# pandegroup/openmm

Hardware: NVIDIA H100
Metric: ns/day (higher is better)
Workload: dtype f32

## Files before the change

### openmm_b200/csrc/engine.cu

```cuda
#include "engine.h"
#include "../../include/b200md.h"
#include <stdexcept>
#include <algorithm>
#include <cmath>
#include <cstring>
#include <cstdlib>
#include <map>
#include <set>
#include <dlfcn.h>
#include <thread>

static std::string g_create_error;

template <class T> struct DevBuf {
    T* p = nullptr; size_t n = 0; bool owned = true;
    void attach(void* ptr, size_t count) { free(); p = (T*) ptr; n = count; owned = false; }
    void alloc(size_t count) {
        if (!owned) { if (count > n) throw std::runtime_error("window buffer too small"); return; }
        free(); n = count; if (count) CUDA_CHECK(cudaMalloc(&p, count*sizeof(T)));
    }
    void upload(const std::vector<T>& v) { if (v.size() > n) alloc(v.size()); if (!v.empty()) CUDA_CHECK(cudaMemcpy(p, v.data(), v.size()*sizeof(T), cudaMemcpyHostToDevice)); }
    void zero() { if (n) CUDA_CHECK(cudaMemset(p, 0, n*sizeof(T))); }
    void free() { if (p && owned) cudaFree(p); p = nullptr; n = 0; owned = true; }
    ~DevBuf() { free(); }
// ... 39 lines not shown
    bool pmeOnly = false;
    bool listDirty = true;
    bool overlapPme = true;
    bool pmeBrick = true;
    int brickAtoms = 64, brickPoints = 8192;
    bool listBuilt = false;
    std::vector<double> mass, charge, sigma, epsilon;
    b200md_nonbonded_desc nbdesc{};
    bool haveNb = false;
    std::vector<int> excI, excJ; std::vector<double> excQQ, excSig, excEps;
    std::vector<int> bondI, bondJ; std::vector<double> bondR0, bondK;
    std::vector<int> angI, angJ, angK; std::vector<double> angT0, angKK;
    std::vector<int> torI, torJ, torK, torL, torN; std::vector<double> torPhase, torKK;
    std::vector<int> rbI, rbJ, rbK, rbL; std::vector<double> rbC;
    std::vector<int> cmapSize, cmapMap, cmapAtoms; std::vector<double> cmapCoeff;
    std::vector<unsigned char> bondGroup, angGroup, torGroup, rbGroup, cmapGroup;
    std::vector<int> conI, conJ; std::vector<double> conD;
    int cmFreq = 0;
    std::vector<int4> hUnitAtoms;
    double boxA[3] = {0, 0, 0}, boxB[3] = {0, 0, 0}, boxC[3] = {0, 0, 0};
    bool haveBox = false;
    bool haveOrigin = false;
    double padFrac = 0.10;
    DevBuf<float4> posq, velm, sposq[2], swrap[2], refPos, atomShift, blockCenter[2], blockHalf[2], superCenter[2], superHalf[2];
    DevBuf<float2> sigeps, ssigeps[2];
    DevBuf<double> chargeD; DevBuf<double2> sigepsD;
    DevBuf<long long> force;
    DevBuf<double> energy, cmScratch;
    DevBuf<int> molStart, molAtoms, cellOffset, sorig[2], sortedOf, cellRank, cellCount, cellFill, atomCell, tmpSorted, tileI[2], tileJ[2], tileMask[2], listCounters, counters, exclStart, exclList;
    DevBuf<unsigned int> maskPool[2];
    DevBuf<unsigned long long> stepCounter;
    DevBuf<unsigned int> blocksDone;
    bool stepStateValid = false;
    DevBuf<real> grid, eterm;
    DevBuf<long long> gridFixed;
    DevBuf<real2> cgrid;
    DevBuf<real2> tw[3];
    DevBuf<double> moduli[3];
    DevBuf<int2> bondAtoms, excAtoms; DevBuf<double2> bondParams, angleParams;
    DevBuf<int4> angleAtoms, torsionAtoms, unitAtoms; DevBuf<double4> torsionParams, excParams;
    DevBuf<int> unitType; DevBuf<float4> unitParams;
    DevBuf<unsigned char> bondGroupDev, angGroupDev, torGroupDev, rbGroupDev, cmapGroupDev;
    DevBuf<int4> rbAtoms, cmapAtomsDev; DevBuf<double> rbParams, cmapCoeffDev; DevBuf<int> cmapMapDev; DevBuf<int2> cmapMapsDev;
    std::vector<int> ccmaCons;
    DevBuf<int> ccCompCon, ccCompAtom, ccRowStart, ccCol, ccAtoms, ccAStart, ccACon;
    DevBuf<int2> ccConAtoms; DevBuf<float> ccDist, ccRedMass, ccVal, ccDelta1, ccDelta2;
    DevBuf<float4> ccRij, ccXold, ccXunc;
    int precision = B200MD_PRECISION_SINGLE;
    DevBuf<float4> posqCorr; DevBuf<double4> velmD, unitParamsD;
    DevBuf<double> ccDistD, ccRedMassD, ccDelta1D, ccDelta2D; DevBuf<double4> ccRijD, ccXoldD, ccXuncD, ccXposD;
    bool mixed() const { return precision == B200MD_PRECISION_MIXED; }
    CcmaDev ccma{};
    NbDev nb{};
    PmeDev pme{};
    BondedDev bd{};
    UnitDev units{};
    IntegDev integ{};
    bool haveIntegrator = false;
    double dt = 0, temperature = 0, friction = 0;
    double time = 0;
    int64_t stepCount = 0;
    double selfEnergy = 0, dispersionCoefficient = 0;
    int64_t forceEvals = 0, kernelLaunches = 0, graphInstantiations = 0;
    DevBuf<int> baroStart, baroAtoms;
    int baroNmol = 0;
    DevBuf<float4> savePosq, savePosqCorr; DevBuf<int> saveCellOffset; DevBuf<long long> saveForce;
// ... 1018 lines not shown
    c->cellOffset.alloc((size_t) 3*NP); c->cellOffset.zero();
    nb.cellOffset = c->cellOffset.p; nb.nmol = 0; nb.molStart = nullptr; nb.molAtoms = nullptr;
    if ((nb.method == B200MD_NB_CUTOFF_PERIODIC || nb.method == B200MD_NB_PME) && c->world == 1 && !c->pmeOnly) {
        std::vector<int> parent(N);
        for (int i = 0; i < N; i++) parent[i] = i;
        auto find = [&](int x) { while (parent[x] != x) { parent[x] = parent[parent[x]]; x = parent[x]; } return x; };
        auto join = [&](int a, int b) { a = find(a); b = find(b); if (a != b) parent[std::max(a, b)] = std::min(a, b); };
        for (size_t i = 0; i < c->bondI.size(); i++) join(c->bondI[i], c->bondJ[i]);
        for (size_t i = 0; i < c->angI.size(); i++) { join(c->angI[i], c->angJ[i]); join(c->angJ[i], c->angK[i]); }
        for (size_t i = 0; i < c->torI.size(); i++) { join(c->torI[i], c->torJ[i]); join(c->torJ[i], c->torK[i]); join(c->torK[i], c->torL[i]); }
        for (size_t i = 0; i < c->rbI.size(); i++) { join(c->rbI[i], c->rbJ[i]); join(c->rbJ[i], c->rbK[i]); join(c->rbK[i], c->rbL[i]); }
        for (size_t i = 0; i < c->cmapAtoms.size(); i++) join(c->cmapAtoms[i - i%8], c->cmapAtoms[i]);
        for (size_t i = 0; i < c->conI.size(); i++) join(c->conI[i], c->conJ[i]);
        for (size_t i = 0; i < c->excI.size(); i++) join(c->excI[i], c->excJ[i]);
        std::vector<int> molOf(N), count;
        std::map<int, int> id;
        for (int i = 0; i < N; i++) {
            const int r = find(i);
            auto it = id.find(r);
            if (it == id.end()) { it = id.insert(std::make_pair(r, (int) count.size())).first; count.push_back(0); }
            molOf[i] = it->second; count[it->second]++;
        }
        std::vector<int> start(count.size() + 1, 0), fill(count.size(), 0), atoms(N);
        for (size_t m = 0; m < count.size(); m++) start[m+1] = start[m] + count[m];
        for (int i = 0; i < N; i++) atoms[start[molOf[i]] + fill[molOf[i]]++] = i;
        c->molStart.upload(start); c->molAtoms.upload(atoms);
        nb.nmol = (int) count.size(); nb.molStart = c->molStart.p; nb.molAtoms = c->molAtoms.p;
    }
    if (nb.method == B200MD_NB_PME) setup_pme(c, c->nbdesc.grid[0], c->nbdesc.grid[1], c->nbdesc.grid[2], c->nbdesc.ewald_alpha);
    if (fft_beside_tiles(c)) pair_set_carveout(fft_cta_smem_bytes(c->pme), sizeof(long long)*(size_t) c->brickPoints + 64);
    c->finalized = true;
    try { apply_box(c); } catch (...) { c->finalized = false; throw; }
    c->integ.stepCounter = c->stepCounter.p;
    c->integ.fused = 0; c->integ.cmEveryStep = 0; c->integ.cmScratch = c->cmScratch.p; c->integ.blocksDone = c->blocksDone.p;
    API_END(ctx)
}

extern "C" int b200md_update_nonbonded_params(b200md_ctx* ctx, const double* q, const double* sig, const double* eps,
                                              int nexc, const double* eqq, const double* esig, const double* eeps, double dispCoef) {
    API_BEGIN(ctx)
    require(ctx->finalized, "update params before finalize");
    require(nexc == (int) ctx->excI.size(), "update_nonbonded_params: the number of exceptions cannot change");
    ctx->charge.assign(q, q + ctx->natoms); ctx->sigma.assign(sig, sig + ctx->natoms); ctx->epsilon.assign(eps, eps + ctx->natoms);
    if (nexc) { ctx->excQQ.assign(eqq, eqq+nexc); ctx->excSig.assign(esig, esig+nexc); ctx->excEps.assign(eeps, eeps+nexc); }
    ctx->dispersionCoefficient = dispCoef;
    CUDA_CHECK(cudaStreamSynchronize(ctx->stream));
    upload_params(ctx);
    const int one = 1;
    CUDA_CHECK(cudaMemcpy(&ctx->counters.p[CT_REBUILD], &one, sizeof(int), cudaMemcpyHostToDevice)); ctx->listDirty = true;
    invalidate_graph(ctx);
    API_END(ctx)
}

extern "C" int b200md_update_bonded_params(b200md_ctx* ctx, int kind, int n, const double* a, const double* b, const int* periodicity) {
    API_BEGIN(ctx)
    require(ctx->finalized, "update_bonded_params before finalize");
    CUDA_CHECK(cudaStreamSynchronize(ctx->stream));
    if (kind == 0) {
        require(n == ctx->bd.nbonds, "the number of bonds cannot change");
        std::vector<double2> p(n); for (int i = 0; i < n; i++) p[i] = make_double2(a[i], b[i]);
        ctx->bondParams.upload(p);
    }
    else if (kind == 1) {
        require(n == ctx->bd.nangles, "the number of angles cannot change");
        std::vector<double2> p(n); for (int i = 0; i < n; i++) p[i] = make_double2(a[i], b[i]);
        ctx->angleParams.upload(p);
    }
// ... 212 lines not shown
    const char* p = (const char*) buf + sizeof(h);
    CUDA_CHECK(cudaMemcpy(ctx->posq.p, p, sizeof(float4)*ctx->npad, cudaMemcpyHostToDevice)); p += sizeof(float4)*ctx->npad;
    if (ctx->mixed()) {
        CUDA_CHECK(cudaMemcpy(ctx->posqCorr.p, p, sizeof(float4)*ctx->npad, cudaMemcpyHostToDevice)); p += sizeof(float4)*ctx->npad;
        CUDA_CHECK(cudaMemcpy(ctx->velmD.p, p, sizeof(double4)*ctx->npad, cudaMemcpyHostToDevice)); p += sizeof(double4)*ctx->npad;
    }
    else { CUDA_CHECK(cudaMemcpy(ctx->velm.p, p, sizeof(float4)*ctx->npad, cudaMemcpyHostToDevice)); p += sizeof(float4)*ctx->npad; }
    CUDA_CHECK(cudaMemcpy(ctx->cellOffset.p, p, sizeof(int)*3*ctx->npad, cudaMemcpyHostToDevice));
    CUDA_CHECK(cudaMemcpy(ctx->stepCounter.p, &h.rngStep, sizeof(unsigned long long), cudaMemcpyHostToDevice));
    host_set_state(ctx); ctx->velStale = false;
    if (ctx->haveBox) apply_box(ctx);
    const int one = 1;
    CUDA_CHECK(cudaMemcpy(&ctx->counters.p[CT_REBUILD], &one, sizeof(int), cudaMemcpyHostToDevice)); ctx->listDirty = true;
    API_END(ctx)
}

static bool role_split(const b200md_ctx* c) { return c->world > 1 && c->comm && !c->p2p && c->nb.method == B200MD_NB_PME && c->haveNb; }
static NbDev role_nb(const b200md_ctx* c) {
    NbDev nb = c->nb;
    if (role_split(c)) {
        if (c->rank == c->world - 1) { nb.rank = 0; nb.world = 1; }
        else nb.world = c->world - 1;
    }
    return nb;
}

static PmeDev pme_for_launch(const b200md_ctx* c) {
    PmeDev p = c->pme;
    p.brickAtoms = (c->pmeBrick && c->world == 1 && !c->pmeOnly && c->listBuilt) ? c->brickAtoms : 0;
    p.brickPoints = c->brickPoints;
    return p;
}

static int enqueue_forces(b200md_ctx* c, int terms, bool energy, bool forcesAlreadyZero = false, bool inStep = false, unsigned int groupMask = 0xffffffffu) {
    int launches = 0;
    cudaStream_t s = c->stream;
    if (!forcesAlreadyZero) CUDA_CHECK(cudaMemsetAsync(c->force.p, 0, sizeof(long long)*3*c->npad, s));
    if (energy) CUDA_CHECK(cudaMemsetAsync(c->energy.p, 0, sizeof(double)*B200MD_NUM_ENERGY, s));
    bool direct = (terms & B200MD_TERM_NB_DIRECT) && c->haveNb;
    bool recip = (terms & B200MD_TERM_NB_RECIP) && c->haveNb && c->nb.method == B200MD_NB_PME;
    const bool split = role_split(c);
    const int pmeRank = c->world - 1;
    NbDev nbSave = c->nb;
    if (split) {
        if (c->rank == pmeRank) direct = false; else recip = false;
        c->nb = role_nb(c);
    }
    struct Restore { b200md_ctx* c; NbDev saved; ~Restore() { c->nb = saved; } } restore{c, nbSave};
    const bool p2p = c->p2p;
    const bool fork = direct && recip && c->overlapPme && !(c->world > 1 && c->comm && !p2p);
    cudaStream_t sp = fork ? c->streamPme : s;
    if (p2p && !direct) { launch_pos_wait(c->nb, c->cd, s); launches++; }
    const PmeDev pme = pme_for_launch(c);
    const bool forkAfterList = fork && direct && pme.brickAtoms > 0;
    auto launch_recip = [&]() {
        if (fork) {
            CUDA_CHECK(cudaEventRecord(c->evFork, s));
            CUDA_CHECK(cudaStreamWaitEvent(sp, c->evFork, 0));
        }
        if (recip) {
            launch_pme_spread(c->nb, pme, c->cd, sp); launches++;
            if (p2p) { launch_grid_push(c->pme, c->cd, sp); launches++; }
            else if (c->world > 1 && c->comm && !split) {
                int rc = g_nccl.AllReduce(c->gridFixed.p, c->gridFixed.p, (size_t) c->pme.nx*c->pme.ny*c->pme.nz, NCCL_INT64, NCCL_SUM, c->comm, sp);
                if (rc != 0) throw std::runtime_error("ncclAllReduce(grid) failed");
            }
            launch_pme_fft_conv(c->nb, c->pme, c->cd, energy && (split || p2p || c->rank == 0), fft_beside_tiles(c), sp); launches += pme_fft_launch_count(c->pme);
            launch_pme_gather(c->nb, pme, c->cd, sp); launches++;
        }
        if (fork) CUDA_CHECK(cudaEventRecord(c->evJoin, sp));
    };
    if (!forkAfterList) launch_recip();
    if (direct) {
        launch_check_displacement(c->nb, c->cd, s); launches++;
        launch_list_build(c->nb, s); launches += LIST_BUILD_LAUNCHES;
    }
    int bterms = terms & (B200MD_TERM_BONDS | B200MD_TERM_ANGLES | B200MD_TERM_TORSIONS | B200MD_TERM_RB_TORSIONS | B200MD_TERM_CMAP);
    if (c->haveNb) bterms |= terms & B200MD_TERM_NB_DIRECT;
    const int nbonded = c->bd.nbonds + c->bd.nangles + c->bd.ntorsions + c->bd.nrb + c->bd.ncmap + c->bd.nexc;
    const bool bonded = bterms && nbonded > 0 && !(split && c->rank == pmeRank);
    auto launch_bonded_terms = [&](cudaStream_t sb) { BondedDev bd = c->bd; bd.groupMask = groupMask; launch_bonded(c->nb, bd, bterms, energy, sb); launches++; };
    const bool forkBonded = forkAfterList && bonded;
    if (forkAfterList) launch_recip();
    if (forkBonded) {
        CUDA_CHECK(cudaStreamWaitEvent(c->streamBonded, c->evFork, 0));
        launch_bonded_terms(c->streamBonded);
        CUDA_CHECK(cudaEventRecord(c->evJoinBonded, c->streamBonded));
    }
    if (direct) { launch_pair(c->nb, energy, s); launches++; }
    if (bonded && !forkBonded) launch_bonded_terms(s);
    const bool pushEarly = p2p && fork;
    if (pushEarly) { launch_force_push(c->nb, c->cd, s); launches++; }
    if (fork) CUDA_CHECK(cudaStreamWaitEvent(s, c->evJoin, 0));
    if (forkBonded) CUDA_CHECK(cudaStreamWaitEvent(s, c->evJoinBonded, 0));
    if (p2p) {
        if (!pushEarly) { launch_force_push(c->nb, c->cd, s); launches++; }
        if (!inStep) { launch_force_total(c->nb, c->cd, s); launches += 2; }
    }
    if (c->world > 1 && c->comm) {
        int rc = 0;
        if (!p2p) rc = g_nccl.AllReduce(c->force.p, c->force.p, (size_t) 3*c->npad, NCCL_INT64, NCCL_SUM, c->comm, s);
        if (rc != 0) throw std::runtime_error("ncclAllReduce(force) failed");
        if (energy) {
            rc = g_nccl.AllReduce(c->energy.p, c->energy.p, B200MD_NUM_ENERGY, NCCL_FLOAT64, NCCL_SUM, c->comm, s);
            if (rc != 0) throw std::runtime_error("ncclAllReduce(energy) failed");
        }
    }
// ... 71 lines not shown
        if (terms & B200MD_TERM_ANGLES) e += h[EN_ANGLE];
        if (terms & B200MD_TERM_TORSIONS) e += h[EN_TORSION];
        if (terms & B200MD_TERM_RB_TORSIONS) e += h[EN_RBTORSION];
        if (terms & B200MD_TERM_CMAP) e += h[EN_CMAP];
        if (ctx->haveNb) {
            if (terms & B200MD_TERM_NB_DIRECT) {
                e += h[EN_NB] + h[EN_EXC];
                const int m = ctx->nb.method;
                if (m == B200MD_NB_CUTOFF_PERIODIC || m == B200MD_NB_PME)
                    e += ctx->dispersionCoefficient/ctx->nb.box.volume;
            }
            if ((terms & B200MD_TERM_NB_RECIP) && ctx->nb.method == B200MD_NB_PME) e += h[EN_RECIP] + ctx->selfEnergy;
        }
        *energy = e;
    }
    API_END(ctx)
}

extern "C" int b200md_set_integrator(b200md_ctx* ctx, int kind, double dt, double temperature, double friction, int seed, double tol) {
    API_BEGIN(ctx)
    require(kind >= 0 && kind <= 2, "unknown integrator kind");
    IntegDev& in = ctx->integ;
    in.kind = kind; in.dt = (float) dt; in.tol = (float) tol; in.seed = (unsigned int) seed;
    const double kT = B200MD_BOLTZ*temperature;
    in.kT = (float) kT;
    const double vscale = std::exp(-dt*friction);
    in.vscale = (float) vscale;
    in.fscale = (float) (friction == 0 ? dt : (1-vscale)/friction);
    in.noisescale = (float) (kind == B200MD_INT_LANGEVIN_MIDDLE ? std::sqrt(1-vscale*vscale) : std::sqrt(kT*(1-vscale*vscale)));
    in.dtD = dt; in.tolD = tol; in.kTD = kT; in.vscaleD = vscale;
    in.fscaleD = friction == 0 ? dt : (1-vscale)/friction;
    in.noisescaleD = kind == B200MD_INT_LANGEVIN_MIDDLE ? std::sqrt(1-vscale*vscale) : std::sqrt(kT*(1-vscale*vscale));
    in.stepCounter = ctx->stepCounter.p;
    in.fused = 0; in.cmEveryStep = 0; in.cmScratch = ctx->cmScratch.p; in.blocksDone = ctx->blocksDone.p;
    ctx->dt = dt; ctx->temperature = temperature; ctx->friction = friction;
    ctx->haveIntegrator = true;
    invalidate_graph(ctx);
    API_END(ctx)
}

static int enqueue_step(b200md_ctx* c) {
    int launches = enqueue_forces(c, B200MD_TERM_ALL, false, true, true);
    IntegDev in = c->integ;
    in.fused = 1;
    in.cmEveryStep = (c->cmFreq == 1) ? 1 : 0;
    in.cmScratch = c->cmScratch.p;
    in.blocksDone = c->blocksDone.p;
    if (c->ccma.ncomp > 0) { launch_ccma_step(c->nb, c->ccma, in, c->stream); launches += 1; }
    launch_integrate(c->nb, c->units, in, c->cd, c->stream); launches += 1;
    return launches;
}

extern "C" int b200md_integrate_only(b200md_ctx* ctx) {
    API_BEGIN(ctx)
    ctx->stepStateValid = false;
    require(ctx->finalized && ctx->haveIntegrator, "integrate before finalize / set_integrator");
    if (ctx->ccma.ncomp > 0) launch_ccma_step(ctx->nb, ctx->ccma, ctx->integ, ctx->stream);
    launch_integrate(ctx->nb, ctx->units, ctx->integ, ctx->cd, ctx->stream);
    ctx->kernelLaunches += 2;
    ctx->velStale = ctx->p2p;
    ctx->time += ctx->dt; ctx->stepCount++;
    CUDA_CHECK(cudaGetLastError());
    API_END(ctx)
}

static void capture_steps(b200md_ctx* c, int nsteps, cudaGraphExec_t* exec, int* launches) {
    cudaGraph_t g;
    CUDA_CHECK(cudaStreamBeginCapture(c->stream, cudaStreamCaptureModeThreadLocal));
    int l = 0;
    try { for (int k = 0; k < nsteps; k++) l += enqueue_step(c); } catch (...) { cudaStreamEndCapture(c->stream, &g); throw; }
    CUDA_CHECK(cudaStreamEndCapture(c->stream, &g));
    *launches = l;
    if (*exec) {
        cudaGraphExecUpdateResultInfo info;
        if (cudaGraphExecUpdate(*exec, g, &info) == cudaSuccess) { cudaGraphDestroy(g); return; }
        (void) cudaGetLastError();
    }
    if (*exec) { cudaGraphExecDestroy(*exec); *exec = nullptr; }
    const cudaError_t e = cudaGraphInstantiate(exec, g, c->world == 1 ? cudaGraphInstantiateFlagUseNodePriority : 0);
    cudaGraphDestroy(g);
    CUDA_CHECK(e);
    c->graphInstantiations++;
}

extern "C" int b200md_step(b200md_ctx* ctx, int nsteps) {
    API_BEGIN(ctx)
    require(ctx->finalized && ctx->haveIntegrator, "step before finalize / set_integrator");
    b200md_ctx* c = ctx;
    int remaining = nsteps;
    prepare_list(c);
    if (!c->stepStateValid) {
        CUDA_CHECK(cudaMemsetAsync(c->force.p, 0, sizeof(long long)*3*c->npad, c->stream));
        if (c->cmFreq == 1) {
            IntegDev in = c->integ;
            in.cmScratch = c->cmScratch.p;
            sync_velocities(c);
            launch_cm_prime(c->nb, in, c->cd, c->stream);
        }
        c->stepStateValid = true;
    }
    while (remaining > 0) {
        if (c->cmFreq > 1 && c->stepCount % c->cmFreq == 0) { sync_velocities(c); launch_remove_cm(c->nb, c->cmScratch.p, c->stream); c->kernelLaunches += 2; }
        int done = 1;
        if (c->useGraph) {
            int untilCm = (c->cmFreq > 1) ? (int) (c->cmFreq - c->stepCount % c->cmFreq) : remaining;
            if (c->graphSteps > 1 && remaining >= c->graphSteps && untilCm >= c->graphSteps) {
                if (!c->multiValid) { int l; capture_steps(c, c->graphSteps, &c->multiGraph, &l); c->stepLaunches = l/c->graphSteps; c->multiValid = true; }
                CUDA_CHECK(cudaGraphLaunch(c->multiGraph, c->stream));
                done = c->graphSteps;
            }
            else {
                if (!c->graphValid) { capture_steps(c, 1, &c->stepGraph, &c->stepLaunches); c->graphValid = true; }
                CUDA_CHECK(cudaGraphLaunch(c->stepGraph, c->stream));
            }
            c->kernelLaunches += (int64_t) c->stepLaunches*done;
        }
        else
            c->kernelLaunches += enqueue_step(c);
        c->velStale = c->p2p;
        c->forceEvals += done;
        c->stepCount += done;
        c->time += c->dt*done;
        remaining -= done;
    }
    CUDA_CHECK(cudaGetLastError());
    API_END(ctx)
}

extern "C" int b200md_kinetic_energy(b200md_ctx* ctx, double* ke) {
    API_BEGIN(ctx)
    require(ctx->finalized, "kinetic_energy before finalize");
    const bool shifted = ctx->haveIntegrator && ctx->integ.kind != B200MD_INT_LANGEVIN_MIDDLE;
    const double shift = !shifted ? 0.0 : ctx->mixed() ? 0.5*ctx->integ.dtD : (double) (0.5f*ctx->integ.dt);
    sync_positions(ctx); sync_velocities(ctx);
    CUDA_CHECK(cudaMemsetAsync(ctx->energy.p + EN_KE, 0, sizeof(double), ctx->stream));
    launch_kinetic_energy(ctx->nb, ctx->units, ctx->integ, shift, ctx->stream);
    launch_ccma_kinetic(ctx->nb, ctx->ccma, shift, 1e-4f, ctx->stream);
    ctx->kernelLaunches++;
    CUDA_CHECK(cudaMemcpyAsync(ke, ctx->energy.p + EN_KE, sizeof(double), cudaMemcpyDeviceToHost, ctx->stream));
    check_flags(ctx);
    API_END(ctx)
}
extern "C" int b200md_apply_constraints(b200md_ctx* ctx, double tol) {
    API_BEGIN(ctx)
    sync_positions(ctx);
    launch_constrain_positions(ctx->nb, ctx->units, tol, ctx->stream);
    launch_ccma_apply(ctx->nb, ctx->ccma, false, tol, ctx->stream);
    ctx->kernelLaunches++;
    CUDA_CHECK(cudaStreamSynchronize(ctx->stream));
    API_END(ctx)
}
extern "C" int b200md_apply_velocity_constraints(b200md_ctx* ctx, double tol) {
    API_BEGIN(ctx)
    ctx->stepStateValid = false;
    sync_positions(ctx); sync_velocities(ctx);
    launch_constrain_velocities(ctx->nb, ctx->units, tol, ctx->stream);
    launch_ccma_apply(ctx->nb, ctx->ccma, true, tol, ctx->stream);
    ctx->kernelLaunches++;
    CUDA_CHECK(cudaStreamSynchronize(ctx->stream));
    API_END(ctx)
}

extern "C" int b200md_comm_unique_id(void* id128) {
    std::string err;
    if (!g_nccl.load(err)) { g_create_error = err; return -1; }
    return g_nccl.GetUniqueId(id128) == 0 ? 0 : -1;
}
extern "C" int b200md_comm_init(b200md_ctx* ctx, int rank, int world, const void* id128) {
    API_BEGIN(ctx)
    require(!ctx->finalized, "comm_init must precede finalize");
    require(!ctx->mixed() || world <= 1, "comm_init: mixed precision is not supported in multi-GPU runs (use Precision=single)");
    std::string err;
    if (!g_nccl.load(err)) throw std::runtime_error(err);
    NcclApi::Uid uid; memcpy(uid.b, id128, 128);
    int rc = g_nccl.CommInitRank(&ctx->comm, world, uid, rank);
    if (rc != 0) throw std::runtime_error(std::string("ncclCommInitRank failed: ") + (g_nccl.GetErrorString ? g_nccl.GetErrorString(rc) : "?"));
    ctx->rank = rank; ctx->world = world;
// ... 171 lines not shown
```

### openmm_b200/csrc/engine.h

```cpp
#pragma once
#include <cuda_runtime.h>
#include <stdint.h>
#include <stdexcept>
#include <string>
#include <vector>

#define B200MD_TILE 32
#define B200MD_PME_ORDER 5
#define B200MD_FORCE_SCALE 4294967296.0
#define B200MD_ONE_4PI_EPS0 138.93545764438198
#define B200MD_BOLTZ 0.00831446261815324
#define B200MD_MAX_RADIX 16
#define B200MD_MAX_FFT_STAGES 8

#define CUDA_CHECK(x) do { cudaError_t e_ = (x); if (e_ != cudaSuccess) throw std::runtime_error(std::string(#x) + ": " + cudaGetErrorString(e_)); } while (0)

template <typename... P, typename... A>
inline void launch_high(void (*kernel)(P...), dim3 grid, dim3 block, size_t smem, cudaStream_t s, A... args) {
    static const int hi = [] { int lo = 0, h = 0; cudaDeviceGetStreamPriorityRange(&lo, &h); return h; }();
    cudaLaunchAttribute at[1];
    at[0].id = cudaLaunchAttributePriority;
    at[0].val.priority = hi;
    cudaLaunchConfig_t cfg = {};
    cfg.gridDim = grid; cfg.blockDim = block; cfg.dynamicSmemBytes = smem; cfg.stream = s;
// ... 111 lines not shown

struct BondedDev {
    int nbonds, nangles, ntorsions, nrb, ncmap, nexc;
    const int2* bondAtoms; const double2* bondParams;
    const int4* angleAtoms; const double2* angleParams;
    const int4* torsionAtoms; const double4* torsionParams;
    const int4* rbAtoms; const double* rbParams;
    const int4* cmapAtoms; const int* cmapMap; const int2* cmapMaps; const double* cmapCoeff;
    const int2* excAtoms; const double4* excParams;
    int excPeriodic;
    const unsigned char* bondGroup; const unsigned char* angleGroup; const unsigned char* torsionGroup;
    const unsigned char* rbGroup; const unsigned char* cmapGroup;
    unsigned int groupMask;
};

struct UnitDev {
    int nunits;
    const int4* unitAtoms;
    const int* unitType;
    const float4* unitParams;
    const double4* unitParamsD;
};

struct IntegDev {
    int kind;
    float dt, vscale, fscale, noisescale;
    float kT;
    float tol;
    double dtD, vscaleD, fscaleD, noisescaleD, kTD, tolD;
    unsigned int seed;
    unsigned long long stepIndex;
    unsigned long long* stepCounter;
    int fused;
    int cmEveryStep;
    double* cmScratch;
    unsigned int* blocksDone;
};

#define B200MD_MAX_RANKS 8
enum { CH_POS = 0,
       CH_FORCE = 1,
       CH_FINAL = 2,
       CH_GRID = 3,
       CH_FWD = 4,
       CH_INV = 5,
       CH_POT = 6,
       CH_VEL = 7,
       CH_COUNT = 8 };
struct CommDev {
    int rank, world;
    int atomLo[B200MD_MAX_RANKS + 1];
    int unitLo[B200MD_MAX_RANKS + 1];
    int xLo[B200MD_MAX_RANKS + 1];
    int lineChunk;
    int maxPlanes;
    char* peer[B200MD_MAX_RANKS];
    size_t offFlags, offPosq, offVelm, offForce, offFinbox, offCm, offGridInbox, offLineBuf, offPlaneBuf, offGrid;
    unsigned long long* epoch;
    unsigned long long* posNeed;
    unsigned int* done;
    int* errFlag;
    int posByPush;
};

#ifdef __CUDACC__
__device__ __forceinline__ unsigned long long ld_acquire_sys(const unsigned long long* p) {
// ... 48 lines not shown
    return q;
}
#endif

#ifdef __CUDACC__
__device__ __forceinline__ float fixed_to_float(long long v) {
    const int hi = (int) (v >> 32);
    const unsigned int lo = (unsigned int) v;
    return __int2float_rn(hi) + __uint2float_rn(lo)*2.3283064365386963e-10f;
}
__device__ __forceinline__ long long float_to_fixed(float f) {
    const float fl = floorf(f);
    const int hi = __float2int_rd(f);
    const unsigned int lo = __float2uint_rz((f - fl)*4294967296.0f);
    return ((long long) hi << 32) | (long long) lo;
}

__host__ __device__ __forceinline__ void pos_split(double x, float& hi, float& lo) { hi = (float) x; lo = (float) (x - (double) hi); }
__host__ __device__ __forceinline__ double pos_join(float hi, float lo) { return (double) hi + (double) lo; }
template <class R> struct Vec4Of;
template <> struct Vec4Of<float> { typedef float4 T; };
template <> struct Vec4Of<double> { typedef double4 T; };
template <class R> using R4 = typename Vec4Of<R>::T;

__device__ __forceinline__ float4 make_r4(float x, float y, float z, float w) { return make_float4(x, y, z, w); }
__device__ __forceinline__ double4 make_r4(double x, double y, double z, double w) { return make_double4(x, y, z, w); }

template <class R> __device__ R4<R> load_pos(const NbDev& nb, int a);
template <> __device__ __forceinline__ float4 load_pos<float>(const NbDev& nb, int a) { return nb.posq[a]; }
template <> __device__ __forceinline__ double4 load_pos<double>(const NbDev& nb, int a) {
    const float4 h = nb.posq[a], l = nb.posqCorr[a];
    return make_double4(pos_join(h.x, l.x), pos_join(h.y, l.y), pos_join(h.z, l.z), (double) h.w);
}
template <class R> __device__ void store_pos(const NbDev& nb, int a, R x, R y, R z);
template <> __device__ __forceinline__ void store_pos<float>(const NbDev& nb, int a, float x, float y, float z) {
    nb.posq[a] = make_float4(x, y, z, nb.posq[a].w);
}
template <> __device__ __forceinline__ void store_pos<double>(const NbDev& nb, int a, double x, double y, double z) {
    float hx, hy, hz, lx, ly, lz;
    pos_split(x, hx, lx); pos_split(y, hy, ly); pos_split(z, hz, lz);
    nb.posq[a] = make_float4(hx, hy, hz, nb.posq[a].w);
    nb.posqCorr[a] = make_float4(lx, ly, lz, 0.f);
}
template <class R> __device__ R4<R>* vel_array(const NbDev& nb);
template <> __device__ __forceinline__ float4* vel_array<float>(const NbDev& nb) { return nb.velm; }
template <> __device__ __forceinline__ double4* vel_array<double>(const NbDev& nb) { return nb.velmD; }

template <class R> __device__ R fixed_to_real(long long v);
template <> __device__ __forceinline__ float fixed_to_real<float>(long long v) { return fixed_to_float(v); }
template <> __device__ __forceinline__ double fixed_to_real<double>(long long v) { return (double) v*(1.0/B200MD_FORCE_SCALE); }

__device__ __forceinline__ float rsqrt_r(float x) { return rsqrtf(x); }
__device__ __forceinline__ double rsqrt_r(double x) { return rsqrt(x); }
__device__ __forceinline__ float sqrt_r(float x) { return sqrtf(x); }
__device__ __forceinline__ double sqrt_r(double x) { return sqrt(x); }
__device__ __forceinline__ float fabs_r(float x) { return fabsf(x); }
__device__ __forceinline__ double fabs_r(double x) { return fabs(x); }
#endif

template <class R> struct IntegR { R dt, vscale, fscale, noisescale, kT, tol; };
#ifdef __CUDACC__
template <class R> __device__ IntegR<R> integ_r(const IntegDev& in);
template <> __device__ __forceinline__ IntegR<float> integ_r<float>(const IntegDev& in) { return {in.dt, in.vscale, in.fscale, in.noisescale, in.kT, in.tol}; }
template <> __device__ __forceinline__ IntegR<double> integ_r<double>(const IntegDev& in) { return {in.dtD, in.vscaleD, in.fscaleD, in.noisescaleD, in.kTD, in.tolD}; }
#endif

struct CcmaDev {
    int ncomp, ncon, natomsC;
    const int* compConStart;
    const int* compAtomStart;
    const int2* conAtoms;
    const float* conDist;
    const float* conRedMass;
    const int* rowStart; const int* col; const float* val;
    const int* atoms;
// ... 89 lines not shown
```

### openmm_b200/csrc/integrate.cu

```cuda
#include "engine.h"
#include <algorithm>
#include "../../include/b200md.h"

template <class R> struct V3 { R x, y, z; };
template <class R> __device__ __forceinline__ V3<R> operator+(V3<R> a, V3<R> b) { return {a.x+b.x, a.y+b.y, a.z+b.z}; }
template <class R> __device__ __forceinline__ V3<R> operator-(V3<R> a, V3<R> b) { return {a.x-b.x, a.y-b.y, a.z-b.z}; }
template <class R> __device__ __forceinline__ V3<R> operator*(V3<R> a, R s) { return {a.x*s, a.y*s, a.z*s}; }
template <class R> __device__ __forceinline__ R dot(V3<R> a, V3<R> b) { return a.x*b.x + a.y*b.y + a.z*b.z; }

template <class R>
__device__ void settle_positions(const V3<R>* x, V3<R>* d, const R* m, R dist1, R dist2) {
    const V3<R> xp0 = d[0], xp1 = d[1], xp2 = d[2];
    const R xb0 = x[1].x-x[0].x, yb0 = x[1].y-x[0].y, zb0 = x[1].z-x[0].z;
    const R xc0 = x[2].x-x[0].x, yc0 = x[2].y-x[0].y, zc0 = x[2].z-x[0].z;
    const R invTotalMass = R(1)/(m[0]+m[1]+m[2]);
    const R xcom = (xp0.x*m[0] + (xb0+xp1.x)*m[1] + (xc0+xp2.x)*m[2])*invTotalMass;
    const R ycom = (xp0.y*m[0] + (yb0+xp1.y)*m[1] + (yc0+xp2.y)*m[2])*invTotalMass;
    const R zcom = (xp0.z*m[0] + (zb0+xp1.z)*m[1] + (zc0+xp2.z)*m[2])*invTotalMass;
    const R xa1 = xp0.x - xcom, ya1 = xp0.y - ycom, za1 = xp0.z - zcom;
    const R xb1 = xb0 + xp1.x - xcom, yb1 = yb0 + xp1.y - ycom, zb1 = zb0 + xp1.z - zcom;
    const R xc1 = xc0 + xp2.x - xcom, yc1 = yc0 + xp2.y - ycom, zc1 = zc0 + xp2.z - zcom;
    const R xaksZd = yb0*zc0 - zb0*yc0, yaksZd = zb0*xc0 - xb0*zc0, zaksZd = xb0*yc0 - yb0*xc0;
    const R xaksXd = ya1*zaksZd - za1*yaksZd, yaksXd = za1*xaksZd - xa1*zaksZd, zaksXd = xa1*yaksZd - ya1*xaksZd;
    const R xaksYd = yaksZd*zaksXd - zaksZd*yaksXd, yaksYd = zaksZd*xaksXd - xaksZd*zaksXd, zaksYd = xaksZd*yaksXd - yaksZd*xaksXd;
// ... 146 lines not shown
            }
            U.f[k] = {fixed_to_real<R>(fx), fixed_to_real<R>(fy), fixed_to_real<R>(fz)};
        }
    }
    return true;
}

template <class R>
__device__ __forceinline__ void constrain_pos(const Unit<R>& U, V3<R>* d, R tol) {
    if (U.type == 1) settle_positions(U.x, d, U.m, U.prm.x, U.prm.y);
    else if (U.type == 2) { const R dist[3] = {U.prm.x, U.prm.y, U.prm.z}; shake_positions(U.x, d, U.invM, dist, U.n-1, tol); }
}
template <class R>
__device__ __forceinline__ void constrain_vel(const Unit<R>& U, V3<R>* v, R tol) {
    if (U.type == 1) settle_velocities(U.x, v, U.m);
    else if (U.type == 2) shake_velocities(U.x, v, U.invM, U.n-1, tol);
}

template <int KIND, class R>
__global__ void __launch_bounds__(128, sizeof(R) == 8 ? 1 : 0) k_integrate(NbDev nb, UnitDev un, IntegDev in, CommDev cd) {
    const bool multi = cd.world > 1;
    const bool useInbox = multi && in.fused;
    const unsigned long long E = multi ? *cd.epoch + 1ull : 0ull;
    if (useInbox) comm_wait(cd, CH_FORCE, E);
    const int u = (multi ? cd.unitLo[cd.rank] : 0) + blockIdx.x*blockDim.x + threadIdx.x;
    const bool active = u < (multi ? cd.unitLo[cd.rank + 1] : un.nunits);
    const unsigned long long step = *in.stepCounter;
    const IntegR<R> ic = integ_r<R>(in);
    Unit<R> U;
    U.n = 0;
    V3<R> d[4];
    const R invDt = R(1)/ic.dt;
    const bool cmFused = in.fused && in.cmEveryStep;
    V3<R> vcm = {R(0), R(0), R(0)};
    if (cmFused) {
        double c[4];
        if (multi) {
            const double* t = (const double*) (cd.peer[cd.rank] + cd.offCm) + 4*(step % 3ull);
            c[0] = c[1] = c[2] = c[3] = 0.0;
            for (int q = 0; q < cd.world; q++) for (int k = 0; k < 4; k++) c[k] += t[q*12 + k];
        }
        else { const double* t = in.cmScratch + 4*(step % 3ull); c[0] = t[0]; c[1] = t[1]; c[2] = t[2]; c[3] = t[3]; }
        const double im = (c[3] > 0.0) ? 1.0/c[3] : 0.0;
        vcm = {(R) (c[0]*im), (R) (c[1]*im), (R) (c[2]*im)};
    }
    if (active) {
    load_unit(nb, un, u, U, true, useInbox ? &cd : nullptr);
    if (in.fused) {
        _Pragma("unroll") for (int k = 0; k < 4; k++) if (k < U.n) {
            const int a = U.atom[k];
            nb.force[a] = 0; nb.force[a + nb.npad] = 0; nb.force[a + 2*nb.npad] = 0;
            if (U.invM[k] > R(0)) U.v[k] = U.v[k] - vcm;
        }
    }
    if (KIND == B200MD_INT_LANGEVIN_MIDDLE) {
        _Pragma("unroll") for (int k = 0; k < 4; k++) if (k < U.n) U.v[k] = U.v[k] + U.f[k]*(ic.dt*U.invM[k]);
        constrain_vel(U, U.v, ic.tol);
        V3<R> du[4];
        _Pragma("unroll") for (int k = 0; k < 4; k++) if (k < U.n) {
            d[k] = U.v[k]*(R(0.5)*ic.dt);
            if (U.invM[k] > R(0)) {
                const float3 g = gauss3(in.seed, U.atom[k], step);
                const R ns = ic.noisescale*sqrt_r(ic.kT*U.invM[k]);
                U.v[k] = U.v[k]*ic.vscale + V3<R>{g.x, g.y, g.z}*ns;
            }
            d[k] = d[k] + U.v[k]*(R(0.5)*ic.dt);
            if (U.invM[k] == R(0)) d[k] = {R(0), R(0), R(0)};
            du[k] = d[k];
        }
        constrain_pos(U, d, ic.tol);
        _Pragma("unroll") for (int k = 0; k < 4; k++) if (k < U.n) U.v[k] = U.v[k] + (d[k] - du[k])*invDt;
    }
    else {
        _Pragma("unroll") for (int k = 0; k < 4; k++) if (k < U.n) {
            V3<R> vn;
            if (KIND == B200MD_INT_LANGEVIN) {
                vn = U.v[k]*ic.vscale + U.f[k]*(ic.fscale*U.invM[k]);
                if (U.invM[k] > R(0) && ic.noisescale > R(0)) {
                    const float3 g = gauss3(in.seed, U.atom[k], step);
                    vn = vn + V3<R>{g.x, g.y, g.z}*(ic.noisescale*sqrt_r(U.invM[k]));
                }
            }
            else
                vn = U.v[k] + U.f[k]*(ic.dt*U.invM[k]);
            if (U.invM[k] == R(0)) vn = U.v[k];
            d[k] = (U.invM[k] == R(0)) ? V3<R>{R(0), R(0), R(0)} : vn*ic.dt;
        }
        constrain_pos(U, d, ic.tol);
        _Pragma("unroll") for (int k = 0; k < 4; k++) if (k < U.n) if (U.invM[k] > R(0)) U.v[k] = d[k]*invDt;
    }
    _Pragma("unroll") for (int k = 0; k < 4; k++) if (k < U.n) {
        const int a = U.atom[k];
        store_pos<R>(nb, a, U.x[k].x + d[k].x, U.x[k].y + d[k].y, U.x[k].z + d[k].z);
        vel_array<R>(nb)[a] = make_r4(U.v[k].x, U.v[k].y, U.v[k].z, U.invM[k]);
        if (multi && !cd.posByPush) {
            const float4 pn = nb.posq[a];
            for (int k = 1; k < cd.world; k++) {
                const int q = (cd.rank + k) % cd.world;
                ((float4*) (cd.peer[q] + cd.offPosq))[a] = pn;
            }
        }
    }
    }
    if (!in.fused && !(multi && !cd.posByPush)) return;
    if (cmFused) {
        double px = 0, py = 0, pz = 0, m = 0;
        _Pragma("unroll") for (int k = 0; k < 4; k++) if (k < U.n && U.invM[k] > R(0)) {
            const double mk = U.m[k];
            px += mk*U.v[k].x; py += mk*U.v[k].y; pz += mk*U.v[k].z; m += mk;
        }
        for (int off = 16; off > 0; off >>= 1) {
            px += __shfl_xor_sync(0xffffffffu, px, off); py += __shfl_xor_sync(0xffffffffu, py, off);
            pz += __shfl_xor_sync(0xffffffffu, pz, off); m += __shfl_xor_sync(0xffffffffu, m, off);
        }
        __shared__ double red[4][4];
        if ((threadIdx.x & 31) == 0) { red[threadIdx.x >> 5][0] = px; red[threadIdx.x >> 5][1] = py; red[threadIdx.x >> 5][2] = pz; red[threadIdx.x >> 5][3] = m; }
        __syncthreads();
        if (threadIdx.x < 4) {
            double t = 0;
            for (int w = 0; w < (int) (blockDim.x >> 5); w++) t += red[w][threadIdx.x];
            atomicAdd(&in.cmScratch[4*((step + 1ull) % 3ull) + threadIdx.x], t);
            if (blockIdx.x == 0) in.cmScratch[4*((step + 2ull) % 3ull) + threadIdx.x] = 0.0;
        }
    }
    if (multi && !cd.posByPush) {
        const bool lastBlock = comm_arrive(cd, CH_POS, gridDim.x);
        if (lastBlock && threadIdx.x == 0) {
            if (cmFused) {
                const double* mine = in.cmScratch + 4*((step + 1ull) % 3ull);
                for (int q = 0; q < cd.world; q++) {
                    double* t = (double*) (cd.peer[q] + cd.offCm) + cd.rank*12 + 4*((step + 1ull) % 3ull);
                    for (int k = 0; k < 4; k++) t[k] = ((volatile const double*) mine)[k];
                }
            }
            comm_publish(cd, CH_POS, E);
// ... 224 lines not shown
```

### openmm_b200/csrc/nonbonded.cu

```cuda
#include "engine.h"
#include "../../include/b200md.h"
#include <algorithm>

#define FULL 0xffffffffu

__device__ __forceinline__ float3 min_image(float3 d, const BoxDev& b) {
    if (b.triclinic) {
        float s = floorf(d.z*b.invCz + 0.5f);
        d.x -= s*b.cx; d.y -= s*b.cy; d.z -= s*b.cz;
        s = floorf(d.y*b.invBy + 0.5f);
        d.x -= s*b.bx; d.y -= s*b.by;
        s = floorf(d.x*b.invAx + 0.5f);
        d.x -= s*b.ax;
    }
    else {
        d.x -= b.ax*rintf(d.x*b.invAx);
        d.y -= b.by*rintf(d.y*b.invBy);
        d.z -= b.cz*rintf(d.z*b.invCz);
    }
    return d;
}

__device__ __forceinline__ float box_dist2(float3 d, float hx, float hy, float hz, const BoxDev& b, bool periodic) {
    if (periodic) d = min_image(d, b);
    if (!periodic || !b.triclinic) {
        const float dx = fmaxf(0.f, fabsf(d.x) - hx), dy = fmaxf(0.f, fabsf(d.y) - hy), dz = fmaxf(0.f, fabsf(d.z) - hz);
        return dx*dx + dy*dy + dz*dz;
    }
    float best = 3e38f;
    for (int sz = -1; sz <= 1; sz++)
        for (int sy = -1; sy <= 1; sy++)
            for (int sx = -1; sx <= 1; sx++) {
                const float x = d.x + sx*b.ax + sy*b.bx + sz*b.cx;
                const float y = d.y + sy*b.by + sz*b.cy;
                const float z = d.z + sz*b.cz;
                const float dx = fmaxf(0.f, fabsf(x) - hx), dy = fmaxf(0.f, fabsf(y) - hy), dz = fmaxf(0.f, fabsf(z) - hz);
                best = fminf(best, dx*dx + dy*dy + dz*dz);
            }
    return best;
}

__global__ void __launch_bounds__(256) k_check_gather(NbDev nb, CommDev cd) {
    comm_wait(cd, CH_POS, cd.world > 1 ? *cd.posNeed : 0ull);
    const int s = blockIdx.x*blockDim.x + threadIdx.x;
    const ListDev& L = nb.list[nb.counters[CT_CUR] & 1];
    if (s == 0) { nb.counters[CT_CURSOR] = 0; nb.counters[CT_PAIRSTART] = 0; }
    if (s < nb.natoms) {
        const float4 p = nb.posq[s];
        const float4 r = nb.refPos[s];
        const float dx = p.x-r.x, dy = p.y-r.y, dz = p.z-r.z;
        const float d2 = dx*dx + dy*dy + dz*dz;
        if (!(d2 <= nb.halfPad2))
            nb.counters[CT_REBUILD] = 1;
    }
    if (s < nb.npad) {
        int a = L.sorig[s];
        if (a < 0 || a >= nb.natoms) a = L.sorig[nb.natoms-1];
        a = min(max(a, 0), nb.natoms-1);
        float4 p = nb.posq[a];
        if (s >= nb.natoms) p.w = 0.f;
        L.sposq[s] = p;
    }
}

__device__ __forceinline__ void wrap_molecule(const NbDev& nb, int m) {
    const int begin = nb.molStart[m], end = nb.molStart[m+1];
    const float4 p = nb.posq[nb.molAtoms[begin]];
    const double* R = nb.box.recip;
    const double px = p.x - nb.origin[0], py = p.y - nb.origin[1], pz = p.z - nb.origin[2];
    const double f[3] = {px*R[0] + py*R[3] + pz*R[6], px*R[1] + py*R[4] + pz*R[7], px*R[2] + py*R[5] + pz*R[8]};
    int k[3];
    bool move = false;
    for (int d = 0; d < 3; d++) {
        const double w = floor(f[d]);
        k[d] = (w >= 2.0 || w <= -2.0) ? (int) w : 0;
        move |= (k[d] != 0);
    }
    if (!move) return;
    const BoxDev& b = nb.box;
    const double sx = -(k[0]*(double) b.dax + k[1]*(double) b.bx + k[2]*(double) b.cx);
    const double sy = -(k[1]*(double) b.dby + k[2]*(double) b.cy);
    const double sz = -(k[2]*(double) b.dcz);
    for (int t = begin; t < end; t++) {
        const int a = nb.molAtoms[t];
        if (nb.posqCorr) {
// ... 860 lines not shown
```

Baseline: 1383.

## Fold neighbor-list displacement check and sorted-position gather into constraint/integrate kernel

In single-rank runs without CCMA, the per-step displacement check and the gather into sorted positions move into the fused integration kernel. After each atom's position is stored, that kernel tests it against the reference position, writes it into the sorted-position array and resets the list cursors. This removes one kernel launch and a full pass over the positions each step. The cost is extra state tracking (listChecked) so the check runs once before the first step of a call, plus a serial loop that fills the padding atoms in one thread.

```diff
diff --git a/openmm_b200/csrc/engine.cu b/openmm_b200/csrc/engine.cu
--- a/openmm_b200/csrc/engine.cu
+++ b/openmm_b200/csrc/engine.cu
@@ -95,6 +95,7 @@
     DevBuf<unsigned long long> stepCounter;
     DevBuf<unsigned int> blocksDone;
     bool stepStateValid = false;
+    bool listChecked = false;
     DevBuf<real> grid, eterm;
     DevBuf<long long> gridFixed;
     DevBuf<real2> cgrid;
@@ -1179,7 +1180,7 @@
     c->finalized = true;
     try { apply_box(c); } catch (...) { c->finalized = false; throw; }
     c->integ.stepCounter = c->stepCounter.p;
-    c->integ.fused = 0; c->integ.cmEveryStep = 0; c->integ.cmScratch = c->cmScratch.p; c->integ.blocksDone = c->blocksDone.p;
+    c->integ.fused = 0; c->integ.checkList = 0; c->integ.cmEveryStep = 0; c->integ.cmScratch = c->cmScratch.p; c->integ.blocksDone = c->blocksDone.p;
     API_END(ctx)
 }
 
@@ -1458,6 +1459,10 @@
     return p;
 }
 
+static bool fold_list_check(const b200md_ctx* c) {
+    return c->world == 1 && c->haveNb && !c->pmeOnly && c->ccma.ncomp == 0;
+}
+
 static int enqueue_forces(b200md_ctx* c, int terms, bool energy, bool forcesAlreadyZero = false, bool inStep = false, unsigned int groupMask = 0xffffffffu) {
     int launches = 0;
     cudaStream_t s = c->stream;
@@ -1498,7 +1503,7 @@
     };
     if (!forkAfterList) launch_recip();
     if (direct) {
-        launch_check_displacement(c->nb, c->cd, s); launches++;
+        if (!(inStep && fold_list_check(c))) { launch_check_displacement(c->nb, c->cd, s); launches++; }
         launch_list_build(c->nb, s); launches += LIST_BUILD_LAUNCHES;
     }
     int bterms = terms & (B200MD_TERM_BONDS | B200MD_TERM_ANGLES | B200MD_TERM_TORSIONS | B200MD_TERM_RB_TORSIONS | B200MD_TERM_CMAP);
@@ -1636,7 +1641,7 @@
     in.fscaleD = friction == 0 ? dt : (1-vscale)/friction;
     in.noisescaleD = kind == B200MD_INT_LANGEVIN_MIDDLE ? std::sqrt(1-vscale*vscale) : std::sqrt(kT*(1-vscale*vscale));
     in.stepCounter = ctx->stepCounter.p;
-    in.fused = 0; in.cmEveryStep = 0; in.cmScratch = ctx->cmScratch.p; in.blocksDone = ctx->blocksDone.p;
+    in.fused = 0; in.checkList = 0; in.cmEveryStep = 0; in.cmScratch = ctx->cmScratch.p; in.blocksDone = ctx->blocksDone.p;
     ctx->dt = dt; ctx->temperature = temperature; ctx->friction = friction;
     ctx->haveIntegrator = true;
     invalidate_graph(ctx);
@@ -1647,6 +1652,7 @@
     int launches = enqueue_forces(c, B200MD_TERM_ALL, false, true, true);
     IntegDev in = c->integ;
     in.fused = 1;
+    in.checkList = fold_list_check(c) ? 1 : 0;
     in.cmEveryStep = (c->cmFreq == 1) ? 1 : 0;
     in.cmScratch = c->cmScratch.p;
     in.blocksDone = c->blocksDone.p;
@@ -1692,7 +1698,11 @@
     require(ctx->finalized && ctx->haveIntegrator, "step before finalize / set_integrator");
     b200md_ctx* c = ctx;
     int remaining = nsteps;
+    const bool fold = fold_list_check(c);
+    const bool checkFirst = fold && !(c->listChecked && c->stepStateValid && !c->listDirty);
     prepare_list(c);
+    if (checkFirst) { launch_check_displacement(c->nb, c->cd, c->stream); c->kernelLaunches++; }
+    c->listChecked = false;
     if (!c->stepStateValid) {
         CUDA_CHECK(cudaMemsetAsync(c->force.p, 0, sizeof(long long)*3*c->npad, c->stream));
         if (c->cmFreq == 1) {
@@ -1727,6 +1737,7 @@
         c->time += c->dt*done;
         remaining -= done;
     }
+    c->listChecked = fold;
     CUDA_CHECK(cudaGetLastError());
     API_END(ctx)
 }
@@ -1747,6 +1758,7 @@
 }
 extern "C" int b200md_apply_constraints(b200md_ctx* ctx, double tol) {
     API_BEGIN(ctx)
+    ctx->listChecked = false;
     sync_positions(ctx);
     launch_constrain_positions(ctx->nb, ctx->units, tol, ctx->stream);
     launch_ccma_apply(ctx->nb, ctx->ccma, false, tol, ctx->stream);
diff --git a/openmm_b200/csrc/engine.h b/openmm_b200/csrc/engine.h
--- a/openmm_b200/csrc/engine.h
+++ b/openmm_b200/csrc/engine.h
@@ -167,6 +167,7 @@
     unsigned long long stepIndex;
     unsigned long long* stepCounter;
     int fused;
+    int checkList;
     int cmEveryStep;
     double* cmScratch;
     unsigned int* blocksDone;
@@ -281,15 +282,25 @@
     const float4 h = nb.posq[a], l = nb.posqCorr[a];
     return make_double4(pos_join(h.x, l.x), pos_join(h.y, l.y), pos_join(h.z, l.z), (double) h.w);
 }
-template <class R> __device__ void store_pos(const NbDev& nb, int a, R x, R y, R z);
-template <> __device__ __forceinline__ void store_pos<float>(const NbDev& nb, int a, float x, float y, float z) {
-    nb.posq[a] = make_float4(x, y, z, nb.posq[a].w);
-}
-template <> __device__ __forceinline__ void store_pos<double>(const NbDev& nb, int a, double x, double y, double z) {
+template <class R> __device__ float4 store_pos(const NbDev& nb, int a, R x, R y, R z);
+template <> __device__ __forceinline__ float4 store_pos<float>(const NbDev& nb, int a, float x, float y, float z) {
+    const float4 p = make_float4(x, y, z, nb.posq[a].w);
+    nb.posq[a] = p;
+    return p;
+}
+template <> __device__ __forceinline__ float4 store_pos<double>(const NbDev& nb, int a, double x, double y, double z) {
     float hx, hy, hz, lx, ly, lz;
     pos_split(x, hx, lx); pos_split(y, hy, ly); pos_split(z, hz, lz);
-    nb.posq[a] = make_float4(hx, hy, hz, nb.posq[a].w);
+    const float4 p = make_float4(hx, hy, hz, nb.posq[a].w);
+    nb.posq[a] = p;
     nb.posqCorr[a] = make_float4(lx, ly, lz, 0.f);
+    return p;
+}
+
+__device__ __forceinline__ bool moved_beyond_half_padding(float4 p, float4 r, float halfPad2) {
+    const float dx = p.x-r.x, dy = p.y-r.y, dz = p.z-r.z;
+    const float d2 = dx*dx + dy*dy + dz*dz;
+    return !(d2 <= halfPad2);
 }
 template <class R> __device__ R4<R>* vel_array(const NbDev& nb);
 template <> __device__ __forceinline__ float4* vel_array<float>(const NbDev& nb) { return nb.velm; }
diff --git a/openmm_b200/csrc/integrate.cu b/openmm_b200/csrc/integrate.cu
--- a/openmm_b200/csrc/integrate.cu
+++ b/openmm_b200/csrc/integrate.cu
@@ -202,6 +202,11 @@
     V3<R> d[4];
     const R invDt = R(1)/ic.dt;
     const bool cmFused = in.fused && in.cmEveryStep;
+    float4* sposq = nullptr;
+    if (in.checkList) {
+        sposq = (nb.counters[CT_CUR] & 1) ? nb.list[1].sposq : nb.list[0].sposq;
+        if (blockIdx.x == 0 && threadIdx.x == 0) { nb.counters[CT_CURSOR] = 0; nb.counters[CT_PAIRSTART] = 0; }
+    }
     V3<R> vcm = {R(0), R(0), R(0)};
     if (cmFused) {
         double c[4];
@@ -216,6 +221,11 @@
     }
     if (active) {
     load_unit(nb, un, u, U, true, useInbox ? &cd : nullptr);
+    float4 ref[4];
+    int slot[4];
+    if (in.checkList) {
+        _Pragma("unroll") for (int k = 0; k < 4; k++) if (k < U.n) { ref[k] = nb.refPos[U.atom[k]]; slot[k] = nb.sortedOf[U.atom[k]]; }
+    }
     if (in.fused) {
         _Pragma("unroll") for (int k = 0; k < 4; k++) if (k < U.n) {
             const int a = U.atom[k];
@@ -259,10 +269,18 @@
         constrain_pos(U, d, ic.tol);
         _Pragma("unroll") for (int k = 0; k < 4; k++) if (k < U.n) if (U.invM[k] > R(0)) U.v[k] = d[k]*invDt;
     }
+    bool rebuild = false;
     _Pragma("unroll") for (int k = 0; k < 4; k++) if (k < U.n) {
         const int a = U.atom[k];
-        store_pos<R>(nb, a, U.x[k].x + d[k].x, U.x[k].y + d[k].y, U.x[k].z + d[k].z);
+        const float4 p = store_pos<R>(nb, a, U.x[k].x + d[k].x, U.x[k].y + d[k].y, U.x[k].z + d[k].z);
         vel_array<R>(nb)[a] = make_r4(U.v[k].x, U.v[k].y, U.v[k].z, U.invM[k]);
+        if (in.checkList) {
+            rebuild |= moved_beyond_half_padding(p, ref[k], nb.halfPad2);
+            const int s = slot[k];
+            sposq[s] = p;
+            if (s == nb.natoms - 1)
+                for (int t = nb.natoms; t < nb.npad; t++) sposq[t] = make_float4(p.x, p.y, p.z, 0.f);
+        }
         if (multi && !cd.posByPush) {
             const float4 pn = nb.posq[a];
             for (int k = 1; k < cd.world; k++) {
@@ -271,6 +289,7 @@
             }
         }
     }
+    if (rebuild) nb.counters[CT_REBUILD] = 1;
     }
     if (!in.fused && !(multi && !cd.posByPush)) return;
     if (cmFused) {
diff --git a/openmm_b200/csrc/nonbonded.cu b/openmm_b200/csrc/nonbonded.cu
--- a/openmm_b200/csrc/nonbonded.cu
+++ b/openmm_b200/csrc/nonbonded.cu
@@ -46,11 +46,7 @@
     const ListDev& L = nb.list[nb.counters[CT_CUR] & 1];
     if (s == 0) { nb.counters[CT_CURSOR] = 0; nb.counters[CT_PAIRSTART] = 0; }
     if (s < nb.natoms) {
-        const float4 p = nb.posq[s];
-        const float4 r = nb.refPos[s];
-        const float dx = p.x-r.x, dy = p.y-r.y, dz = p.z-r.z;
-        const float d2 = dx*dx + dy*dy + dz*dz;
-        if (!(d2 <= nb.halfPad2))
+        if (moved_beyond_half_padding(nb.posq[s], nb.refPos[s], nb.halfPad2))
             nb.counters[CT_REBUILD] = 1;
     }
     if (s < nb.npad) {
```

New measurement: 1393, median of 6. No clear change (+0.7%).
